# qinliuliuqin/Medical-Segmentation3d-Toolkit

Measured on AMD Instinct MI355X. Metric: patches/sec (96^3, 1-mod V-Net) train-step, higher is better.
Workload: dtype f32; 1 GPU; vnet(1,2) train step (fwd + Dice loss + bwd + fused Adam), 4 patches of 96^3 per GPU, fp32, random-init weights; global_batch=4, patch=96, parallelism=single GPU, wgrad_overlap=True, train_step_hipgraph=False, step_mode=auto, full=False

## Files before the change

### include/seg3d_hip.h

```cpp
#ifndef SEG3D_HIP_H
#define SEG3D_HIP_H

#ifdef __cplusplus
extern "C" {
#endif

#define SEG3D_ABI_VERSION 1

const char* seg3d_last_error(void);
int seg3d_abi_version(void);
const char* seg3d_target_arch(void);
int seg3d_device_count(void);

int seg3d_ncdhw_to_ndhwc(const float* in, float* out, int N, int C, long long S, void* stream);
int seg3d_ndhwc_to_ncdhw(const float* in, float* out, int N, int C, long long S, void* stream);
int seg3d_copy_channels(const float* src, float* dst, long long nvox, int C, int src_ld, int src_off, int dst_ld,
                        int dst_off, void* stream);

int seg3d_pack_weights_tapmajor(const float* w, float* wp, int A, int B, int BP, int T, long long sa, long long sb,
                                int flip, void* stream);
int seg3d_pack_weights_mfma(const float* w, float* wp, int A, int B, int T, long long sa, long long sb, int flip,
                            void* stream);
long long seg3d_packed_mfma_floats(int A, int B, int T);
typedef struct Seg3dPackJob {
// ... 152 lines not shown
                        int C, int relu, int ld_dout , void* stream);
int seg3d_gn_bwd_finalize(const float* part, const float* gamma, const float* mean_rstd, float* abx, float* s12,
                          float* dgamma, float* dbeta, float* dbias, int N, long long S, int C,
                          int acc_mask , void* stream);
int seg3d_gn_bwd_finalize_fused(const float* part, const float* gamma, const float* mean_rstd, float* abx, float* s12,
                                float* dgamma, float* dbeta, float* dbias, int* ticket, int N, long long S, int C,
                                int acc_mask, void* stream);
int seg3d_gn_bwd_apply(const float* dout, const float* out , const float* y, const float* mean_rstd,
                       const float* s12, const float* gamma, const float* beta, float* dy, float* dres, int N, long long S,
                       int C, int relu, int ld_dout , void* stream);

int seg3d_gn_mask_supported(int C);
int seg3d_gn_apply_mask(const float* y, const float* mean_rstd, const float* gamma, const float* beta, const float* res,
                        float* out, unsigned char* mask, int N, long long S, int C, int relu, int ld_out, void* stream);
int seg3d_gn_bwd_reduce_mask(const float* dout, const unsigned char* mask, const float* y, const float* mean_rstd,
                             float* part, int N, long long S, int C, int ld_dout, void* stream);
int seg3d_gn_bwd_apply_mask(const float* dout, const unsigned char* mask, const float* y, const float* mean_rstd,
                            const float* s12, const float* gamma, float* dy, float* dres ,
                            int N, long long S, int C, int ld_dout, void* stream);

int seg3d_gn_apply_mixed(const void* y, const float* mean_rstd, const float* gamma, const float* beta, const void* res,
                         void* out, int N, long long S, int C, int relu, int ld_out, int res_bf16, int out_bf16,
                         int y_bf16, void* stream);
int seg3d_gn_bwd_reduce_bf16(const void* dout_bf16, const void* out_bf16, const void* y, const float* mean_rstd,
                             const float* gamma, const float* beta, float* part, int N, long long S, int C, int relu,
                             int ld_dout, int y_bf16, void* stream);
int seg3d_gn_bwd_apply_bf16(const void* dout_bf16, const void* out_bf16, const void* y, const float* mean_rstd,
                            const float* s12, const float* gamma, const float* beta, void* dy, float* dres, int N,
                            long long S, int C, int relu, int ld_dout, int dy_bf16, int y_bf16, void* stream);

int seg3d_softmax_fwd(const float* in_ndhwc, float* probs_ncdhw, int N, int C, long long S, void* stream);
int seg3d_softmax_bwd(const float* probs_ncdhw, const float* dprobs_ncdhw, float* din_ndhwc, int N, int C, long long S,
                      void* stream);

long long seg3d_dice_blocks(long long S);
int seg3d_dice_fwd(const float* probs, const float* target, const float* weights, float* part, float* sums, float* loss,
                   int N, int C, long long S, void* stream);
int seg3d_dice_bwd(const float* probs, const float* target, const float* sums, const float* weights, const float* gout,
                   float* dprobs, int N, int C, long long S, void* stream);
int seg3d_binary_dice_fwd(const float* probs, const float* target, const float* one, float* part, float* sums, float* loss,
                          int N, long long S, void* stream);
int seg3d_binary_dice_bwd(const float* probs, const float* target, const float* sums, const float* gout, float* dprobs,
                          int N, long long S, void* stream);
long long seg3d_focal_blocks(long long total_vox);
int seg3d_focal_fwd(const float* probs, const float* target, const float* alpha, float* part, float* loss, int N, int C,
                    long long S, long long sn, long long sc, long long ss, float gamma, int size_average, void* stream);
int seg3d_focal_bwd(const float* probs, const float* target, const float* alpha, const float* gout, float* dprobs, int N,
                    int C, long long S, long long sn, long long sc, long long ss, float gamma, int size_average,
                    void* stream);
long long seg3d_compound_loss_part_floats(int N, int C, long long S);
int seg3d_compound_loss_fwd(const float* probs, const float* target, const float* wdice, const float* alpha, float* part,
                            float* coef, float* loss, int N, int C, long long S, float gamma, float dice_weight,
                            float ce_weight, int batch_dice, float ignore_label, void* stream);
int seg3d_compound_loss_bwd(const float* probs, const float* target, const float* coef, const float* alpha,
                            const float* gout, float* dprobs, int N, int C, long long S, float gamma, int batch_dice,
                            float ignore_label, void* stream);

int seg3d_sigmoid_fwd(const float* in_ndhwc, float* probs_ncdhw, int N, int C, long long S, void* stream);
int seg3d_sigmoid_bwd(const float* probs_ncdhw, const float* dprobs_ncdhw, float* din_ndhwc, int N, int C, long long S,
                      void* stream);

int seg3d_ds_head_supported(int Cin, int C);
int seg3d_ds_head_fwd(const float* x, int ldx, const float* w, const float* b, float* probs, int N, long long S, int Cin,
                      int C, void* stream);
long long seg3d_ds_head_bwd_workspace_floats(int N, long long S, int Cin, int C);
int seg3d_ds_head_bwd(const float* probs, const float* dprobs, const float* x, int ldx, const float* w, float* dx, int ld_dx,
// ... 130 lines not shown
```

### medical-segmentation3d-toolkit_amd/segmentation3d/_engine.py

```python
import ctypes
import os

import torch

_HERE = os.path.dirname(os.path.abspath(__file__))
_PKG_ROOT = os.path.dirname(_HERE)
LIB_PATH = os.environ.get('SEG3D_HIP_LIB', os.path.join(_PKG_ROOT, 'lib', 'libseg3d_hip.so'))

_c_int, _c_ll, _c_f, _c_p = ctypes.c_int, ctypes.c_longlong, ctypes.c_float, ctypes.c_void_p


class Normalizer(ctypes.Structure):
    _fields_ = [('type', _c_int), ('mean', _c_f), ('stddev', _c_f), ('clip', _c_int), ('clip_lo', _c_f), ('clip_hi', _c_f)]


class Normalizers(ctypes.Structure):
    _fields_ = [('n', Normalizer * 8)]



class Intensity(ctypes.Structure):
    _fields_ = [('brightness', _c_f), ('contrast', _c_f), ('gamma', _c_f), ('invert', _c_int), ('sigma', _c_f)]


# ... 110 lines not shown
    'seg3d_conv3d_k3_wino2d_wgrad_supported': (_c_int, [_c_int] * 6),
    'seg3d_conv3d_k3_wino2d_wgrad_preferred': (_c_int, [_c_int] * 6),
    'seg3d_conv3d_k3_wino2d_wgrad_workspace_floats': (_c_ll, [_c_int] * 6),
    'seg3d_conv3d_k3_wino2d_wgrad': (_c_int, [_c_p] * 4 + [_c_int] * 7 + [_c_p]),
    'seg3d_conv3d_k3_wino_wgrad_supported': (_c_int, [_c_int] * 6),
    'seg3d_conv3d_k3_wino_wgrad_workspace_floats': (_c_ll, [_c_int] * 6),
    'seg3d_conv3d_k3_wino_wgrad': (_c_int, [_c_p] * 4 + [_c_int] * 7 + [_c_p]),
    'seg3d_conv3d_k3_thin_out_f32mfma_supported': (_c_int, [_c_int] * 2),
    'seg3d_thin_out_f32mfma_packed_floats': (_c_ll, [_c_int] * 2),
    'seg3d_pack_weights_thin_out_f32mfma': (_c_int, [_c_p, _c_p, _c_int, _c_int, _c_ll, _c_ll, _c_int, _c_p]),
    'seg3d_conv3d_k3_thin_out_f32mfma_stats_count': (_c_ll, [_c_int] * 4),
    'seg3d_conv3d_k3_thin_out_f32mfma_fwd': (_c_int, [_c_p] * 5 + [_c_int] * 6 + [_c_p]),
    'seg3d_pack_weights_thin_out': (_c_int, [_c_p, _c_p, _c_int, _c_int, _c_int, _c_ll, _c_ll, _c_int, _c_p]),
    'seg3d_conv3d_k3_thin_out_stats_count': (_c_ll, [_c_int] * 3),
    'seg3d_conv3d_k3_thin_out_fwd': (_c_int, [_c_p] * 5 + [_c_int] * 7 + [_c_p]),
    'seg3d_k3_thin_wgrad_workspace_floats': (_c_ll, [_c_int] * 6),
    'seg3d_k3_thin_wgrad': (_c_int, [_c_p] * 4 + [_c_int] * 6 + [_c_ll, _c_ll, _c_int, _c_int, _c_p]),
    'seg3d_k3_thin_wgrad_fatbf16': (_c_int, [_c_p] * 4 + [_c_int] * 6 + [_c_ll, _c_ll, _c_int, _c_int, _c_p]),
    'seg3d_gn_stats_count': (_c_ll, [_c_ll]),
    'seg3d_gn_stats_partial': (_c_int, [_c_p, _c_p, _c_int, _c_ll, _c_p]),
    'seg3d_gn_stats_finalize': (_c_int, [_c_p, _c_p, _c_int, _c_int, _c_ll, _c_f, _c_p]),
    'seg3d_gn_apply': (_c_int, [_c_p] * 6 + [_c_int, _c_ll, _c_int, _c_int, _c_int, _c_p]),
    'seg3d_gn_bwd_blocks': (_c_ll, [_c_ll]),
    'seg3d_gn_bwd_reduce': (_c_int, [_c_p] * 7 + [_c_int, _c_ll, _c_int, _c_int, _c_int, _c_p]),
    'seg3d_gn_bwd_finalize': (_c_int, [_c_p] * 8 + [_c_int, _c_ll, _c_int, _c_int, _c_p]),
    'seg3d_gn_bwd_finalize_fused': (_c_int, [_c_p] * 9 + [_c_int, _c_ll, _c_int, _c_int, _c_p]),
    'seg3d_gn_bwd_apply': (_c_int, [_c_p] * 9 + [_c_int, _c_ll, _c_int, _c_int, _c_int, _c_p]),
    'seg3d_gn_mask_supported': (_c_int, [_c_int]),
    'seg3d_gn_apply_mask': (_c_int, [_c_p] * 7 + [_c_int, _c_ll, _c_int, _c_int, _c_int, _c_p]),
    'seg3d_gn_bwd_reduce_mask': (_c_int, [_c_p] * 5 + [_c_int, _c_ll, _c_int, _c_int, _c_p]),
    'seg3d_gn_bwd_apply_mask': (_c_int, [_c_p] * 8 + [_c_int, _c_ll, _c_int, _c_int, _c_p]),
    'seg3d_softmax_fwd': (_c_int, [_c_p, _c_p, _c_int, _c_int, _c_ll, _c_p]),
    'seg3d_softmax_bwd': (_c_int, [_c_p, _c_p, _c_p, _c_int, _c_int, _c_ll, _c_p]),
    'seg3d_dice_blocks': (_c_ll, [_c_ll]),
    'seg3d_dice_fwd': (_c_int, [_c_p] * 6 + [_c_int, _c_int, _c_ll, _c_p]),
    'seg3d_dice_bwd': (_c_int, [_c_p] * 6 + [_c_int, _c_int, _c_ll, _c_p]),
    'seg3d_binary_dice_fwd': (_c_int, [_c_p] * 6 + [_c_int, _c_ll, _c_p]),
    'seg3d_binary_dice_bwd': (_c_int, [_c_p] * 5 + [_c_int, _c_ll, _c_p]),
    'seg3d_focal_blocks': (_c_ll, [_c_ll]),
    'seg3d_focal_fwd': (_c_int, [_c_p] * 5 + [_c_int, _c_int, _c_ll, _c_ll, _c_ll, _c_ll, _c_f, _c_int, _c_p]),
    'seg3d_focal_bwd': (_c_int, [_c_p] * 5 + [_c_int, _c_int, _c_ll, _c_ll, _c_ll, _c_ll, _c_f, _c_int, _c_p]),
    'seg3d_compound_loss_part_floats': (_c_ll, [_c_int, _c_int, _c_ll]),
    'seg3d_compound_loss_fwd': (_c_int, [_c_p] * 7 + [_c_int, _c_int, _c_ll, _c_f, _c_f, _c_f, _c_int, _c_f, _c_p]),
    'seg3d_compound_loss_bwd': (_c_int, [_c_p] * 6 + [_c_int, _c_int, _c_ll, _c_f, _c_int, _c_f, _c_p]),
    'seg3d_sigmoid_fwd': (_c_int, [_c_p, _c_p, _c_int, _c_int, _c_ll, _c_p]),
    'seg3d_sigmoid_bwd': (_c_int, [_c_p, _c_p, _c_p, _c_int, _c_int, _c_ll, _c_p]),
    'seg3d_ds_head_supported': (_c_int, [_c_int] * 2),
    'seg3d_ds_head_fwd': (_c_int, [_c_p, _c_int, _c_p, _c_p, _c_p, _c_int, _c_ll, _c_int, _c_int, _c_p]),
    'seg3d_ds_head_bwd_workspace_floats': (_c_ll, [_c_int, _c_ll, _c_int, _c_int]),
    'seg3d_ds_head_bwd': (_c_int, [_c_p] * 3 + [_c_int, _c_p, _c_p, _c_int, _c_p, _c_int, _c_ll, _c_int, _c_int, _c_p]),
    'seg3d_ds_head_bwd_finalize': (_c_int, [_c_p] * 3 + [_c_int, _c_ll, _c_int, _c_int, _c_int, _c_p]),
    'seg3d_label_pyramid': (_c_int, [_c_p] * 4 + [_c_int] * 5 + [_c_p]),
    'seg3d_adam_step': (_c_int, [_c_p] * 4 + [_c_ll, _c_int] + [_c_f] * 6 + [_c_p]),
    'seg3d_adam_step_devstep': (_c_int, [_c_p] * 4 + [_c_ll, _c_p, _c_p] + [_c_f] * 6 + [_c_p]),
    'seg3d_grad_sumsq_part_count': (_c_ll, [_c_ll]),
    'seg3d_grad_sumsq_partial': (_c_int, [_c_p, _c_ll, _c_p, _c_p]),
    'seg3d_optim_prepare': (_c_int, [_c_p, _c_p, _c_p, _c_int, _c_f, _c_f, _c_int, _c_f, _c_int, _c_int, _c_f, _c_f, _c_f,
                                     _c_p]),
    'seg3d_sgd_step_ctl': (_c_int, [_c_p, _c_p, _c_p, _c_ll, _c_p, _c_f, _c_f, _c_int, _c_p]),
    'seg3d_adam_step_ctl': (_c_int, [_c_p] * 4 + [_c_ll, _c_p] + [_c_f] * 4 + [_c_p]),
    'seg3d_patch_stats_blocks': (_c_ll, [_c_int] * 3),
    'seg3d_patch_gather_normalize': (_c_int, [_c_p] * 5 + [_c_int] * 8 + [_c_f, _c_f, _c_int, _c_f, _c_p]),
    'seg3d_patch_stats_mc_doubles': (_c_ll, [_c_int] * 5),
    'seg3d_patch_gather_normalize_mc': (_c_int, [_c_p] * 5 + [_c_int] * 8 + [Normalizers, _c_p]),
    'seg3d_patch_scatter_accumulate': (_c_int, [_c_p] * 5 + [_c_int] * 7 + [_c_ll, _c_p]),
    'seg3d_finalize_argmax': (_c_int, [_c_p, _c_p, _c_p, _c_int, _c_ll, _c_ll, _c_p]),
# ... 102 lines not shown
```

### medical-segmentation3d-toolkit_amd/segmentation3d/_ops.py

```python
import contextlib
import ctypes

import torch

from . import _engine as E
from . import _grad_sink as G

GN_EPS = 1e-5

_KINDS = {'k3': (3, 1, 27, False), 'k2s2': (2, 2, 8, False), 'k1': (1, 1, 1, False), 'convT': (2, 2, 8, True)}

FORCE_DIRECT = False
WINOGRAD = True
WINOGRAD2D = True
STREAM_K = True
_TWO_FORWARDS = 0
RELU_MASK = True


@contextlib.contextmanager
def two_forwards():
    global _TWO_FORWARDS
    _TWO_FORWARDS += 1
    try:
# ... 623 lines not shown
               E.ptr(mask), N, D * H * W_, C, int(relu), ld, E.stream_ptr())
        return out
    if _is_bf16(out) or _is_bf16(resn) or _is_bf16(yn):
        E.call('seg3d_gn_apply_mixed', E.ptr(yn), E.ptr(mean_rstd), E.ptr(gamma), E.ptr(beta), E.ptr(resn), E.ptr(out), N,
               D * H * W_, C, int(relu), ld, int(_is_bf16(resn)), int(_is_bf16(out)), int(_is_bf16(yn)), E.stream_ptr())
        return out
    E.call('seg3d_gn_apply', E.ptr(yn), E.ptr(mean_rstd), E.ptr(gamma), E.ptr(beta), E.ptr(resn), E.ptr(out), N,
           D * H * W_, C, int(relu), ld, E.stream_ptr())
    return out


def _row_stride(t, C):
    if t.is_contiguous():
        return 0
    N, D, H, W_, _ = t.shape
    ld = t.stride(3)
    if t.stride(4) != 1 or ld < C or ld % 4 or t.stride(2) != W_ * ld or t.stride(1) != H * t.stride(2) or \
            t.stride(0) != D * t.stride(1) or (t.storage_offset() % 4):
        raise ValueError('expected a contiguous NDHWC tensor or a channel slice of one')
    return ld


GN_FUSED_FINALIZE = False
_GN_TICKETS = {}


def _gn_ticket(device):
    t = _GN_TICKETS.get(device)
    if t is None:
        t = _GN_TICKETS[device] = torch.zeros(1, dtype=torch.int32, device=device)
    return t


def gn_backward(doutn, outn, yn, mean_rstd, gamma, beta, relu, want_dres, want_dbias=True, sinks=(None, None, None),
                dy_bf16=False, mask=None):
    N, D, H, W_, C = yn.shape
    S = D * H * W_
    nblk = E.query('seg3d_gn_bwd_blocks', S)
    part = _empty((N, nblk, C, 3), yn)
    mask_src = outn if relu else None
    ldd = _row_stride(doutn, C)
    act_bf16 = _is_bf16(doutn)
    if act_bf16 != (_is_bf16(mask_src) if mask_src is not None else act_bf16):
        raise TypeError('GroupNorm backward: gradient and saved output differ in dtype')
    if dy_bf16 and not act_bf16:
        raise TypeError('GroupNorm backward: a bf16 conv gradient needs a bf16 unit output')
    if _is_bf16(yn) and not act_bf16:
        yn = _to_f32(yn)
    y16 = int(_is_bf16(yn))
    if mask is not None:
        if not relu or outn is not None or act_bf16 or y16 or mask.dtype != torch.uint8 or not mask.is_contiguous() or \
                mask.numel() * 4 != yn.numel():
            raise ValueError('GroupNorm backward: the ReLU mask belongs to a fp32 ReLU unit and stands in for its output')
        E.call('seg3d_gn_bwd_reduce_mask', E.ptr(doutn), E.ptr(mask), E.ptr(yn), E.ptr(mean_rstd), E.ptr(part), N, S, C, ldd,
               E.stream_ptr())
    elif act_bf16:
        E.call('seg3d_gn_bwd_reduce_bf16', E.ptr(doutn), E.ptr(mask_src), E.ptr(yn), E.ptr(mean_rstd), E.ptr(gamma),
               E.ptr(beta), E.ptr(part), N, S, C, int(relu), ldd, y16, E.stream_ptr())
    else:
        E.call('seg3d_gn_bwd_reduce', E.ptr(doutn), E.ptr(mask_src), E.ptr(yn), E.ptr(mean_rstd), E.ptr(gamma),
               E.ptr(beta), E.ptr(part), N, S, C, int(relu), ldd, E.stream_ptr())
    abx = _empty((N, C, 3), yn)
    s12 = _empty((N, 2), yn)
    sg, sb_, sc = sinks
    for t in sinks:
        if t is not None and (t.numel() != C or not t.is_contiguous()):
            raise ValueError('GroupNorm gradient destination must be a contiguous [C] tensor')
    dgamma = _empty((C,), yn) if sg is None else sg
    dbeta = _empty((C,), yn) if sb_ is None else sb_
    dbias = (_empty((C,), yn) if sc is None else sc) if want_dbias else None
    acc_mask = (1 if sg is not None else 0) | (2 if sb_ is not None else 0) | (4 if (want_dbias and sc is not None) else 0)
    if GN_FUSED_FINALIZE:
        E.call('seg3d_gn_bwd_finalize_fused', E.ptr(part), E.ptr(gamma), E.ptr(mean_rstd), E.ptr(abx), E.ptr(s12),
               E.ptr(dgamma), E.ptr(dbeta), E.ptr(dbias), E.ptr(_gn_ticket(yn.device)), N, S, C, acc_mask, E.stream_ptr())
    else:
        E.call('seg3d_gn_bwd_finalize', E.ptr(part), E.ptr(gamma), E.ptr(mean_rstd), E.ptr(abx), E.ptr(s12), E.ptr(dgamma),
               E.ptr(dbeta), E.ptr(dbias), N, S, C, acc_mask, E.stream_ptr())
    dy = torch.empty(yn.shape, dtype=torch.bfloat16 if dy_bf16 else torch.float32, device=yn.device)
    dres = torch.empty(yn.shape, dtype=torch.float32, device=yn.device) if want_dres else None
    if mask is not None:
        E.call('seg3d_gn_bwd_apply_mask', E.ptr(doutn), E.ptr(mask), E.ptr(yn), E.ptr(mean_rstd), E.ptr(s12), E.ptr(gamma),
               E.ptr(dy), E.ptr(dres), N, S, C, ldd, E.stream_ptr())
    elif act_bf16:
        E.call('seg3d_gn_bwd_apply_bf16', E.ptr(doutn), E.ptr(mask_src), E.ptr(yn), E.ptr(mean_rstd), E.ptr(s12),
               E.ptr(gamma), E.ptr(beta), E.ptr(dy), E.ptr(dres), N, S, C, int(relu), ldd, int(dy_bf16), y16,
               E.stream_ptr())
    else:
        E.call('seg3d_gn_bwd_apply', E.ptr(doutn), E.ptr(mask_src), E.ptr(yn), E.ptr(mean_rstd), E.ptr(s12), E.ptr(gamma),
               E.ptr(beta), E.ptr(dy), E.ptr(dres), N, S, C, int(relu), ldd, E.stream_ptr())
    return (dy, dres, dgamma if sg is None else None, dbeta if sb_ is None else None,
            dbias if (want_dbias and sc is None) else None)


WGRAD_SIDE_STREAM = True
_SIDE_STREAMS = {}
_SIDE_STREAMS_UNPROBED = {}
SIDE_KEEPALIVE = True
_SIDE_KEEP = {}
_JOIN_QUEUED_FOR = [-1]


def _runs_beside(busy, other, spin_cycles=1500000):
    probe = torch.zeros(1024, device=busy.device)
    votes = 0
    for _ in range(3):
        torch.cuda.synchronize()
        s0, e_busy, e_other = (torch.cuda.Event(enable_timing=True) for _ in range(3))
        s0.record(busy)
        other.wait_event(s0)
        with torch.cuda.stream(busy):
            torch.cuda._sleep(spin_cycles)
        e_busy.record(busy)
        with torch.cuda.stream(other):
            probe.add_(1.0)
        e_other.record(other)
        torch.cuda.synchronize()
        votes += int(s0.elapsed_time(e_other) < 0.5 * s0.elapsed_time(e_busy))
    return votes >= 2


def _side_stream(device):
    st = _SIDE_STREAMS.get(device.index)
    if st is None:
        with torch.cuda.device(device):
# ... 331 lines not shown
        return da, db


def cat_channels(a, b):
    return CatChannelsFunction.apply(a, b)


class SoftmaxFunction(torch.autograd.Function):

    @staticmethod
    def forward(ctx, x):
        E.require_device(x)
        xn = to_ndhwc(x)
        N, D, H, W_, C = xn.shape
        probs = _empty((N, C, D, H, W_), xn)
        E.call('seg3d_softmax_fwd', E.ptr(xn), E.ptr(probs), N, C, D * H * W_, E.stream_ptr())
        ctx.save_for_backward(probs)
        return probs

    @staticmethod
    def backward(ctx, dprobs):
        (probs,) = ctx.saved_tensors
        N, C, D, H, W_ = probs.shape
        dp = dprobs.contiguous()
        din = _empty((N, D, H, W_, C), probs)
        E.call('seg3d_softmax_bwd', E.ptr(probs), E.ptr(dp), E.ptr(din), N, C, D * H * W_, E.stream_ptr())
        return from_ndhwc(din)


def softmax_channels(x):
    return SoftmaxFunction.apply(x)


class SigmoidFunction(torch.autograd.Function):

    @staticmethod
    def forward(ctx, x):
        E.require_device(x)
        if x.dtype != torch.float32:
            raise ValueError('the sigmoid head takes float32 logits, got {} (bf16 activation mode supports up to 15 '
                             'regions)'.format(x.dtype))
        xn = to_ndhwc(x)
        N, D, H, W_, C = xn.shape
        probs = _empty((N, C, D, H, W_), xn)
        E.call('seg3d_sigmoid_fwd', E.ptr(xn), E.ptr(probs), N, C, D * H * W_, E.stream_ptr())
        ctx.save_for_backward(probs)
        return probs

    @staticmethod
    def backward(ctx, dprobs):
        (probs,) = ctx.saved_tensors
        N, C, D, H, W_ = probs.shape
        dp = dprobs.contiguous()
        din = _empty((N, D, H, W_, C), probs)
        E.call('seg3d_sigmoid_bwd', E.ptr(probs), E.ptr(dp), E.ptr(din), N, C, D * H * W_, E.stream_ptr())
        return from_ndhwc(din)


def sigmoid_channels(x):
    return SigmoidFunction.apply(x)


class DiceLossFunction(torch.autograd.Function):

    @staticmethod
    def forward(ctx, probs, target, weights):
# ... 229 lines not shown
```

### medical-segmentation3d-toolkit_amd/segmentation3d/network/module/vnet_outblock.py

```python
import torch.nn as nn

from segmentation3d.network.module.layers import Sigmoid, Softmax, attach_unit, run_unit

_FIRST, _SECOND = ('conv1', 'gn1', 'act1'), ('conv2', 'gn2', None)
ACTIVATIONS = ('softmax', 'sigmoid')


def check_activation(activation):
    if activation not in ACTIVATIONS:
        raise ValueError("unknown output activation {!r}: 'softmax' or 'sigmoid'".format(activation))
    return activation


class OutputBlock(nn.Module):

    def __init__(self, in_channels, out_channels, activation='softmax'):
        super(OutputBlock, self).__init__()
        self.activation = check_activation(activation)
        attach_unit(self, _FIRST, 'k3', in_channels, out_channels)
        attach_unit(self, _SECOND, 'k1', out_channels, out_channels, act=False)
        if self.activation == 'sigmoid':
            self.sigmoid = Sigmoid()
        else:
            self.softmax = Softmax(dim=1)

    def forward(self, input):
        hidden = run_unit(self, _FIRST, input, relu=True)
        logits = run_unit(self, _SECOND, hidden, relu=False)
        return self.sigmoid(logits) if self.activation == 'sigmoid' else self.softmax(logits)
```

Measured before the change: 286.4 patches/s.

## Fuse V-Net output block GN/ReLU/1x1 conv/GN/softmax into custom head-tail kernels

Adds HIP kernels that fuse the output block's tail (GN1 apply + ReLU, 1x1 conv, GN2 stats/apply, softmax) and its backward into a few streaming passes. Intermediate activations are recomputed from y1 rather than stored. The aim is to cut memory traffic and kernel launches at full resolution. The cost is extra recompute in each backward pass and extra code paths, limited to at most 8 classes in fp32.

```diff
diff --git a/include/seg3d_hip.h b/include/seg3d_hip.h
--- a/include/seg3d_hip.h
+++ b/include/seg3d_hip.h
@@ -208,6 +208,24 @@
 int seg3d_softmax_fwd(const float* in_ndhwc, float* probs_ncdhw, int N, int C, long long S, void* stream);
 int seg3d_softmax_bwd(const float* probs_ncdhw, const float* dprobs_ncdhw, float* din_ndhwc, int N, int C, long long S,
                       void* stream);
+
+long long seg3d_head_tail_blocks(long long S);
+int seg3d_head_tail_stats(const float* y1, const float* mean_rstd1, const float* gamma1, const float* beta1, const float* w2,
+                          const float* b2, float* stats_partial, int N, long long S, int C, void* stream);
+int seg3d_head_tail_fwd(const float* y1, const float* mean_rstd1, const float* gamma1, const float* beta1, const float* w2,
+                        const float* b2, const float* mean_rstd2, const float* gamma2, const float* beta2, float* probs, int N,
+                        long long S, int C, void* stream);
+int seg3d_head_tail_bwd_stats2(const float* probs, const float* dprobs, const float* y1, const float* mean_rstd1,
+                               const float* gamma1, const float* beta1, const float* w2, const float* b2,
+                               const float* mean_rstd2, float* part2, int N, long long S, int C, void* stream);
+int seg3d_head_tail_bwd_stats1(const float* probs, const float* dprobs, const float* y1, const float* mean_rstd1,
+                               const float* gamma1, const float* beta1, const float* w2, const float* b2,
+                               const float* mean_rstd2, const float* gamma2, const float* s12_2, float* part1, float* wpart,
+                               float* dw2, int N, long long S, int C, int accumulate, void* stream);
+int seg3d_head_tail_bwd_apply(const float* probs, const float* dprobs, const float* y1, const float* mean_rstd1,
+                              const float* gamma1, const float* beta1, const float* w2, const float* b2,
+                              const float* mean_rstd2, const float* gamma2, const float* s12_2, const float* s12_1, float* dy1,
+                              int N, long long S, int C, void* stream);
 
 long long seg3d_dice_blocks(long long S);
 int seg3d_dice_fwd(const float* probs, const float* target, const float* weights, float* part, float* sums, float* loss,
diff --git a/medical-segmentation3d-toolkit_amd/csrc/head_tail.hip b/medical-segmentation3d-toolkit_amd/csrc/head_tail.hip
--- /dev/null
+++ b/medical-segmentation3d-toolkit_amd/csrc/head_tail.hip
@@ -0,0 +1,517 @@
+#include "seg3d_common.h"
+#include "seg3d_hip.h"
+
+#define HT_MAXC 8
+
+template <int C>
+struct HtUnit {
+  float mean1, rstd1, g1[C], b1[C];
+  float w2[C][C], bias2[C];
+  float mean2, rstd2, g2[C], b2[C];
+  __device__ __forceinline__ void load1(const float* __restrict__ mr1, const float* __restrict__ gamma1,
+                                        const float* __restrict__ beta1, const float* __restrict__ w,
+                                        const float* __restrict__ bias, int n) {
+    mean1 = mr1[2 * n], rstd1 = mr1[2 * n + 1];
+#pragma unroll
+    for (int k = 0; k < C; ++k) {
+      g1[k] = gamma1[k], b1[k] = beta1[k];
+      bias2[k] = bias ? bias[k] : 0.f;
+#pragma unroll
+      for (int j = 0; j < C; ++j) w2[k][j] = w[k * C + j];
+    }
+  }
+  __device__ __forceinline__ void load2(const float* __restrict__ mr2, const float* __restrict__ gamma2,
+                                        const float* __restrict__ beta2, int n) {
+    mean2 = mr2[2 * n], rstd2 = mr2[2 * n + 1];
+#pragma unroll
+    for (int c = 0; c < C; ++c) g2[c] = gamma2 ? gamma2[c] : 1.f, b2[c] = beta2 ? beta2[c] : 0.f;
+  }
+};
+
+template <int C>
+__device__ __forceinline__ void ht_a1(const HtUnit<C>& u, const float (&y)[C], float (&a1)[C]) {
+#pragma unroll
+  for (int k = 0; k < C; ++k) a1[k] = fmaxf((y[k] - u.mean1) * u.rstd1 * u.g1[k] + u.b1[k], 0.f);
+}
+template <int C>
+__device__ __forceinline__ void ht_z(const HtUnit<C>& u, const float (&a1)[C], float (&z)[C]) {
+#pragma unroll
+  for (int c = 0; c < C; ++c) z[c] = u.bias2[c];
+#pragma unroll
+  for (int k = 0; k < C; ++k)
+#pragma unroll
+    for (int c = 0; c < C; ++c) z[c] = fmaf(a1[k], u.w2[c][k], z[c]);
+}
+template <int C>
+__device__ __forceinline__ void ht_probs(const HtUnit<C>& u, const float (&z)[C], float (&p)[C]) {
+  float mx = -INFINITY;
+#pragma unroll
+  for (int c = 0; c < C; ++c) {
+    p[c] = (z[c] - u.mean2) * u.rstd2 * u.g2[c] + u.b2[c];
+    mx = fmaxf(mx, p[c]);
+  }
+  float sum = 0.f;
+#pragma unroll
+  for (int c = 0; c < C; ++c) {
+    p[c] = expf(p[c] - mx);
+    sum += p[c];
+  }
+#pragma unroll
+  for (int c = 0; c < C; ++c) p[c] = p[c] / sum;
+}
+template <int C>
+__device__ __forceinline__ void ht_dzn(const float (&p)[C], const float (&dp)[C], float (&dzn)[C]) {
+  float dot = 0.f;
+#pragma unroll
+  for (int c = 0; c < C; ++c) dot += p[c] * dp[c];
+#pragma unroll
+  for (int c = 0; c < C; ++c) dzn[c] = p[c] * (dp[c] - dot);
+}
+template <int C>
+__device__ __forceinline__ void ht_dz(const HtUnit<C>& u, const float (&z)[C], const float (&dzn)[C], float s1, float s2,
+                                      float (&dz)[C]) {
+#pragma unroll
+  for (int c = 0; c < C; ++c) dz[c] = u.rstd2 * (u.g2[c] * dzn[c] - s1 - (z[c] - u.mean2) * u.rstd2 * s2);
+}
+template <int C>
+__device__ __forceinline__ void ht_g1(const HtUnit<C>& u, const float (&a1)[C], const float (&dz)[C], float (&g1)[C]) {
+#pragma unroll
+  for (int k = 0; k < C; ++k) g1[k] = 0.f;
+#pragma unroll
+  for (int c = 0; c < C; ++c)
+#pragma unroll
+    for (int k = 0; k < C; ++k) g1[k] = fmaf(dz[c], u.w2[c][k], g1[k]);
+#pragma unroll
+  for (int k = 0; k < C; ++k) g1[k] = a1[k] > 0.f ? g1[k] : 0.f;
+}
+
+template <int C, bool VEC>
+__device__ __forceinline__ void ht_load_rows(const float* __restrict__ p, int nv, float (&v)[4][C]) {
+  if (VEC) {
+#pragma unroll
+    for (int i = 0; i < C; ++i) {
+      const seg3d_f32x4 t = __builtin_nontemporal_load(reinterpret_cast<const seg3d_f32x4*>(p) + i);
+#pragma unroll
+      for (int j = 0; j < 4; ++j) v[(4 * i + j) / C][(4 * i + j) % C] = t[j];
+    }
+  } else {
+#pragma unroll
+    for (int j = 0; j < 4; ++j)
+#pragma unroll
+      for (int c = 0; c < C; ++c) v[j][c] = j < nv ? p[j * C + c] : 0.f;
+  }
+}
+template <int C, bool VEC>
+__device__ __forceinline__ void ht_store_rows(float* __restrict__ p, int nv, const float (&v)[4][C]) {
+  if (VEC) {
+#pragma unroll
+    for (int i = 0; i < C; ++i) {
+      seg3d_f32x4 t;
+#pragma unroll
+      for (int j = 0; j < 4; ++j) t[j] = v[(4 * i + j) / C][(4 * i + j) % C];
+      __builtin_nontemporal_store(t, reinterpret_cast<seg3d_f32x4*>(p) + i);
+    }
+  } else {
+#pragma unroll
+    for (int j = 0; j < 4; ++j)
+#pragma unroll
+      for (int c = 0; c < C; ++c)
+        if (j < nv) p[j * C + c] = v[j][c];
+  }
+}
+template <int C, bool VEC>
+__device__ __forceinline__ void ht_load_planes(const float* __restrict__ p, i64 S, int nv, float (&v)[4][C]) {
+#pragma unroll
+  for (int c = 0; c < C; ++c) {
+    if (VEC) {
+      const seg3d_f32x4 t = __builtin_nontemporal_load(reinterpret_cast<const seg3d_f32x4*>(p + c * S));
+#pragma unroll
+      for (int j = 0; j < 4; ++j) v[j][c] = t[j];
+    } else {
+#pragma unroll
+      for (int j = 0; j < 4; ++j) v[j][c] = j < nv ? p[c * S + j] : 0.f;
+    }
+  }
+}
+template <int C, bool VEC>
+__device__ __forceinline__ void ht_store_planes(float* __restrict__ p, i64 S, int nv, const float (&v)[4][C]) {
+#pragma unroll
+  for (int c = 0; c < C; ++c) {
+    if (VEC) {
+      const seg3d_f32x4 t = {v[0][c], v[1][c], v[2][c], v[3][c]};
+      __builtin_nontemporal_store(t, reinterpret_cast<seg3d_f32x4*>(p + c * S));
+    } else {
+#pragma unroll
+      for (int j = 0; j < 4; ++j)
+        if (j < nv) p[c * S + j] = v[j][c];
+    }
+  }
+}
+
+struct HtRange {
+  i64 q0, q1;
+  __device__ __forceinline__ HtRange(i64 S, int qpb) {
+    const i64 Q = (S + 3) >> 2;
+    q0 = (i64)blockIdx.x * qpb;
+    q1 = q0 + qpb < Q ? q0 + qpb : Q;
+  }
+};
+template <bool VEC>
+__device__ __forceinline__ int ht_nvalid(i64 S, i64 s) {
+  return VEC ? 4 : (S - s < 4 ? (int)(S - s) : 4);
+}
+
+template <int NV>
+__device__ __forceinline__ void ht_block_sum(float (&v)[NV], double* red) {
+  const int lane = threadIdx.x & 63, wave = threadIdx.x >> 6;
+#pragma unroll
+  for (int k = 0; k < NV; ++k) {
+    const double w = wave_sum_d((double)v[k]);
+    if (lane == 0) red[wave * NV + k] = w;
+  }
+  __syncthreads();
+  if (threadIdx.x == 0) {
+#pragma unroll
+    for (int k = 0; k < NV; ++k) v[k] = (float)((red[k] + red[NV + k]) + (red[2 * NV + k] + red[3 * NV + k]));
+  }
+}
+
+template <int C, bool VEC>
+__global__ __launch_bounds__(256) void head_tail_stats_kernel(const float* __restrict__ y1, const float* __restrict__ mr1,
+                                                                const float* __restrict__ gamma1,
+                                                                const float* __restrict__ beta1, const float* __restrict__ w2,
+                                                                const float* __restrict__ bias2, float* __restrict__ part,
+                                                                i64 S, int qpb) {
+  __shared__ double red[4 * 2];
+  const int n = blockIdx.y;
+  HtUnit<C> u;
+  u.load1(mr1, gamma1, beta1, w2, bias2, n);
+  const HtRange r(S, qpb);
+  float acc[2] = {0.f, 0.f};
+  for (i64 q = r.q0 + threadIdx.x; q < r.q1; q += 256) {
+    const i64 s = 4 * q;
+    const int nv = ht_nvalid<VEC>(S, s);
+    float y[4][C];
+    ht_load_rows<C, VEC>(y1 + ((i64)n * S + s) * C, nv, y);
+#pragma unroll
+    for (int j = 0; j < 4; ++j) {
+      float a1[C], z[C];
+      ht_a1<C>(u, y[j], a1);
+      ht_z<C>(u, a1, z);
+      if (j < nv) {
+#pragma unroll
+        for (int c = 0; c < C; ++c) {
+          acc[0] += z[c];
+          acc[1] += z[c] * z[c];
+        }
+      }
+    }
+  }
+  ht_block_sum<2>(acc, red);
+  if (threadIdx.x == 0) {
+    float* dst = part + ((i64)n * gridDim.x + blockIdx.x) * 2;
+    dst[0] = acc[0];
+    dst[1] = acc[1];
+  }
+}
+
+template <int C, bool VEC>
+__global__ __launch_bounds__(256) void head_tail_fwd_kernel(const float* __restrict__ y1, const float* __restrict__ mr1,
+                                                              const float* __restrict__ gamma1, const float* __restrict__ beta1,
+                                                              const float* __restrict__ w2, const float* __restrict__ bias2,
+                                                              const float* __restrict__ mr2, const float* __restrict__ gamma2,
+                                                              const float* __restrict__ beta2, float* __restrict__ probs, i64 S,
+                                                              int qpb) {
+  const int n = blockIdx.y;
+  HtUnit<C> u;
+  u.load1(mr1, gamma1, beta1, w2, bias2, n);
+  u.load2(mr2, gamma2, beta2, n);
+  const HtRange r(S, qpb);
+  for (i64 q = r.q0 + threadIdx.x; q < r.q1; q += 256) {
+    const i64 s = 4 * q;
+    const int nv = ht_nvalid<VEC>(S, s);
+    float y[4][C], p[4][C];
+    ht_load_rows<C, VEC>(y1 + ((i64)n * S + s) * C, nv, y);
+#pragma unroll
+    for (int j = 0; j < 4; ++j) {
+      float a1[C], z[C];
+      ht_a1<C>(u, y[j], a1);
+      ht_z<C>(u, a1, z);
+      ht_probs<C>(u, z, p[j]);
+    }
+    ht_store_planes<C, VEC>(probs + (i64)n * C * S + s, S, nv, p);
+  }
+}
+
+template <int C, bool VEC>
+__global__ __launch_bounds__(256) void head_tail_bwd_stats2_kernel(const float* __restrict__ probs,
+                                                                     const float* __restrict__ dprobs,
+                                                                     const float* __restrict__ y1, const float* __restrict__ mr1,
+                                                                     const float* __restrict__ gamma1,
+                                                                     const float* __restrict__ beta1, const float* __restrict__ w2,
+                                                                     const float* __restrict__ bias2, const float* __restrict__ mr2,
+                                                                     float* __restrict__ part2, i64 S, int qpb) {
+  __shared__ double red[4 * 3 * C];
+  const int n = blockIdx.y;
+  HtUnit<C> u;
+  u.load1(mr1, gamma1, beta1, w2, bias2, n);
+  u.load2(mr2, nullptr, nullptr, n);
+  const HtRange r(S, qpb);
+  float acc[3 * C];
+#pragma unroll
+  for (int k = 0; k < 3 * C; ++k) acc[k] = 0.f;
+  for (i64 q = r.q0 + threadIdx.x; q < r.q1; q += 256) {
+    const i64 s = 4 * q;
+    const int nv = ht_nvalid<VEC>(S, s);
+    float y[4][C], p[4][C], dp[4][C];
+    ht_load_rows<C, VEC>(y1 + ((i64)n * S + s) * C, nv, y);
+    ht_load_planes<C, VEC>(probs + (i64)n * C * S + s, S, nv, p);
+    ht_load_planes<C, VEC>(dprobs + (i64)n * C * S + s, S, nv, dp);
+#pragma unroll
+    for (int j = 0; j < 4; ++j) {
+      float a1[C], z[C], dzn[C];
+      ht_a1<C>(u, y[j], a1);
+      ht_z<C>(u, a1, z);
+      ht_dzn<C>(p[j], dp[j], dzn);
+      if (j < nv) {
+#pragma unroll
+        for (int c = 0; c < C; ++c) {
+          const float zh = (z[c] - u.mean2) * u.rstd2;
+          acc[3 * c + 0] += dzn[c];
+          acc[3 * c + 1] += dzn[c] * zh;
+          acc[3 * c + 2] += zh;
+        }
+      }
+    }
+  }
+  ht_block_sum<3 * C>(acc, red);
+  if (threadIdx.x == 0) {
+    float* dst = part2 + ((i64)n * gridDim.x + blockIdx.x) * C * 3;
+#pragma unroll
+    for (int k = 0; k < 3 * C; ++k) dst[k] = acc[k];
+  }
+}
+
+template <int C, bool VEC>
+__global__ __launch_bounds__(256) void head_tail_bwd_stats1_kernel(const float* __restrict__ probs,
+                                                                     const float* __restrict__ dprobs,
+                                                                     const float* __restrict__ y1, const float* __restrict__ mr1,
+                                                                     const float* __restrict__ gamma1,
+                                                                     const float* __restrict__ beta1, const float* __restrict__ w2,
+                                                                     const float* __restrict__ bias2, const float* __restrict__ mr2,
+                                                                     const float* __restrict__ gamma2,
+                                                                     const float* __restrict__ s12_2, float* __restrict__ part1,
+                                                                     float* __restrict__ wpart, i64 S, int qpb) {
+  constexpr int NV = 3 * C + C * C;
+  __shared__ double red[4 * NV];
+  const int n = blockIdx.y;
+  HtUnit<C> u;
+  u.load1(mr1, gamma1, beta1, w2, bias2, n);
+  u.load2(mr2, gamma2, nullptr, n);
+  const float s1 = s12_2[2 * n], s2 = s12_2[2 * n + 1];
+  const HtRange r(S, qpb);
+  float acc[NV];
+#pragma unroll
+  for (int k = 0; k < NV; ++k) acc[k] = 0.f;
+  for (i64 q = r.q0 + threadIdx.x; q < r.q1; q += 256) {
+    const i64 s = 4 * q;
+    const int nv = ht_nvalid<VEC>(S, s);
+    float y[4][C], p[4][C], dp[4][C];
+    ht_load_rows<C, VEC>(y1 + ((i64)n * S + s) * C, nv, y);
+    ht_load_planes<C, VEC>(probs + (i64)n * C * S + s, S, nv, p);
+    ht_load_planes<C, VEC>(dprobs + (i64)n * C * S + s, S, nv, dp);
+#pragma unroll
+    for (int j = 0; j < 4; ++j) {
+      float a1[C], z[C], dzn[C], dz[C], g1[C];
+      ht_a1<C>(u, y[j], a1);
+      ht_z<C>(u, a1, z);
+      ht_dzn<C>(p[j], dp[j], dzn);
+      ht_dz<C>(u, z, dzn, s1, s2, dz);
+      ht_g1<C>(u, a1, dz, g1);
+      if (j < nv) {
+#pragma unroll
+        for (int k = 0; k < C; ++k) {
+          const float xh = (y[j][k] - u.mean1) * u.rstd1;
+          acc[3 * k + 0] += g1[k];
+          acc[3 * k + 1] += g1[k] * xh;
+          acc[3 * k + 2] += xh;
+        }
+#pragma unroll
+        for (int c = 0; c < C; ++c)
+#pragma unroll
+          for (int k = 0; k < C; ++k) acc[3 * C + c * C + k] += dz[c] * a1[k];
+      }
+    }
+  }
+  ht_block_sum<NV>(acc, red);
+  if (threadIdx.x == 0) {
+    const i64 slot = (i64)n * gridDim.x + blockIdx.x;
+    float* d1 = part1 + slot * C * 3;
+#pragma unroll
+    for (int k = 0; k < 3 * C; ++k) d1[k] = acc[k];
+    float* dw = wpart + slot * (C * C);
+#pragma unroll
+    for (int k = 0; k < C * C; ++k) dw[k] = acc[3 * C + k];
+  }
+}
+
+__global__ __launch_bounds__(256) void head_tail_wreduce_kernel(const float* __restrict__ wpart, float* __restrict__ dw2,
+                                                                  int slots, int NV, int accumulate) {
+  __shared__ double red[256];
+  const int o = blockIdx.x;
+  double s = 0.0;
+  for (int k = threadIdx.x; k < slots; k += 256) s += (double)wpart[(i64)k * NV + o];
+  red[threadIdx.x] = s;
+  __syncthreads();
+#pragma unroll
+  for (int w = 128; w >= 1; w >>= 1) {
+    if ((int)threadIdx.x < w) red[threadIdx.x] += red[threadIdx.x + w];
+    __syncthreads();
+  }
+  if (threadIdx.x == 0) {
+    const float v = (float)red[0];
+    dw2[o] = accumulate ? dw2[o] + v : v;
+  }
+}
+
+template <int C, bool VEC>
+__global__ __launch_bounds__(256) void head_tail_bwd_apply_kernel(const float* __restrict__ probs,
+                                                                    const float* __restrict__ dprobs,
+                                                                    const float* __restrict__ y1, const float* __restrict__ mr1,
+                                                                    const float* __restrict__ gamma1,
+                                                                    const float* __restrict__ beta1, const float* __restrict__ w2,
+                                                                    const float* __restrict__ bias2, const float* __restrict__ mr2,
+                                                                    const float* __restrict__ gamma2,
+                                                                    const float* __restrict__ s12_2,
+                                                                    const float* __restrict__ s12_1, float* __restrict__ dy1,
+                                                                    i64 S, int qpb) {
+  const int n = blockIdx.y;
+  HtUnit<C> u;
+  u.load1(mr1, gamma1, beta1, w2, bias2, n);
+  u.load2(mr2, gamma2, nullptr, n);
+  const float s1 = s12_2[2 * n], s2 = s12_2[2 * n + 1];
+  const float t1 = s12_1[2 * n], t2 = s12_1[2 * n + 1];
+  const HtRange r(S, qpb);
+  for (i64 q = r.q0 + threadIdx.x; q < r.q1; q += 256) {
+    const i64 s = 4 * q;
+    const int nv = ht_nvalid<VEC>(S, s);
+    float y[4][C], p[4][C], dp[4][C], dy[4][C];
+    ht_load_rows<C, VEC>(y1 + ((i64)n * S + s) * C, nv, y);
+    ht_load_planes<C, VEC>(probs + (i64)n * C * S + s, S, nv, p);
+    ht_load_planes<C, VEC>(dprobs + (i64)n * C * S + s, S, nv, dp);
+#pragma unroll
+    for (int j = 0; j < 4; ++j) {
+      float a1[C], z[C], dzn[C], dz[C], g1[C];
+      ht_a1<C>(u, y[j], a1);
+      ht_z<C>(u, a1, z);
+      ht_dzn<C>(p[j], dp[j], dzn);
+      ht_dz<C>(u, z, dzn, s1, s2, dz);
+      ht_g1<C>(u, a1, dz, g1);
+#pragma unroll
+      for (int k = 0; k < C; ++k) dy[j][k] = u.rstd1 * (u.g1[k] * g1[k] - t1 - (y[j][k] - u.mean1) * u.rstd1 * t2);
+    }
+    ht_store_rows<C, VEC>(dy1 + ((i64)n * S + s) * C, nv, dy);
+  }
+}
+
+extern "C" long long seg3d_head_tail_blocks(long long S) { return seg3d_gn_bwd_blocks(S); }
+
+static inline int ht_qpb(i64 S, int nblk) { return (int)((((S + 3) >> 2) + nblk - 1) / nblk); }
+static inline bool ht_aligned(const void* p) { return (reinterpret_cast<unsigned long long>(p) & 15) == 0; }
+
+#define HT_CASE(KERNEL, CC, ...)                                                                             \
+  case CC:                                                                                                   \
+    if (vec) hipLaunchKernelGGL((KERNEL<CC, true>), grid, dim3(256), 0, s, __VA_ARGS__);                     \
+    else hipLaunchKernelGGL((KERNEL<CC, false>), grid, dim3(256), 0, s, __VA_ARGS__);                        \
+    break;
+#define HT_LAUNCH(KERNEL, ...)                                                                               \
+  switch (C) {                                                                                               \
+    HT_CASE(KERNEL, 1, __VA_ARGS__) HT_CASE(KERNEL, 2, __VA_ARGS__) HT_CASE(KERNEL, 3, __VA_ARGS__)          \
+    HT_CASE(KERNEL, 4, __VA_ARGS__) HT_CASE(KERNEL, 5, __VA_ARGS__) HT_CASE(KERNEL, 6, __VA_ARGS__)          \
+    HT_CASE(KERNEL, 7, __VA_ARGS__) HT_CASE(KERNEL, 8, __VA_ARGS__)                                          \
+  }
+#define HT_REQUIRE_SHAPE(name)                                                                               \
+  SEG3D_REQUIRE(N > 0 && N <= 65535 && S > 0, name ": bad arguments");                                       \
+  SEG3D_REQUIRE(C >= 1 && C <= HT_MAXC, name ": classes %d not in [1, %d]", C, HT_MAXC)
+
+extern "C" int seg3d_head_tail_stats(const float* y1, const float* mean_rstd1, const float* gamma1, const float* beta1,
+                                     const float* w2, const float* b2, float* stats_partial, int N, long long S, int C,
+                                     void* stream) {
+  SEG3D_REQUIRE(y1 && mean_rstd1 && gamma1 && beta1 && w2 && stats_partial, "seg3d_head_tail_stats: bad arguments");
+  HT_REQUIRE_SHAPE("seg3d_head_tail_stats");
+  const int nblk = (int)seg3d_head_tail_blocks(S), qpb = ht_qpb(S, nblk);
+  const bool vec = (S & 3) == 0 && ht_aligned(y1);
+  const dim3 grid(nblk, N);
+  hipStream_t s = (hipStream_t)stream;
+  HT_LAUNCH(head_tail_stats_kernel, y1, mean_rstd1, gamma1, beta1, w2, b2, stats_partial, (i64)S, qpb)
+  SEG3D_LAUNCH_CHECK("seg3d_head_tail_stats");
+  return SEG3D_OK;
+}
+
+extern "C" int seg3d_head_tail_fwd(const float* y1, const float* mean_rstd1, const float* gamma1, const float* beta1,
+                                   const float* w2, const float* b2, const float* mean_rstd2, const float* gamma2,
+                                   const float* beta2, float* probs, int N, long long S, int C, void* stream) {
+  SEG3D_REQUIRE(y1 && mean_rstd1 && gamma1 && beta1 && w2 && mean_rstd2 && gamma2 && beta2 && probs,
+                "seg3d_head_tail_fwd: bad arguments");
+  HT_REQUIRE_SHAPE("seg3d_head_tail_fwd");
+  const int nblk = (int)seg3d_head_tail_blocks(S), qpb = ht_qpb(S, nblk);
+  const bool vec = (S & 3) == 0 && ht_aligned(y1) && ht_aligned(probs);
+  const dim3 grid(nblk, N);
+  hipStream_t s = (hipStream_t)stream;
+  HT_LAUNCH(head_tail_fwd_kernel, y1, mean_rstd1, gamma1, beta1, w2, b2, mean_rstd2, gamma2, beta2, probs, (i64)S, qpb)
+  SEG3D_LAUNCH_CHECK("seg3d_head_tail_fwd");
+  return SEG3D_OK;
+}
+
+extern "C" int seg3d_head_tail_bwd_stats2(const float* probs, const float* dprobs, const float* y1, const float* mean_rstd1,
+                                          const float* gamma1, const float* beta1, const float* w2, const float* b2,
+                                          const float* mean_rstd2, float* part2, int N, long long S, int C, void* stream) {
+  SEG3D_REQUIRE(probs && dprobs && y1 && mean_rstd1 && gamma1 && beta1 && w2 && mean_rstd2 && part2,
+                "seg3d_head_tail_bwd_stats2: bad arguments");
+  HT_REQUIRE_SHAPE("seg3d_head_tail_bwd_stats2");
+  const int nblk = (int)seg3d_head_tail_blocks(S), qpb = ht_qpb(S, nblk);
+  const bool vec = (S & 3) == 0 && ht_aligned(y1) && ht_aligned(probs) && ht_aligned(dprobs);
+  const dim3 grid(nblk, N);
+  hipStream_t s = (hipStream_t)stream;
+  HT_LAUNCH(head_tail_bwd_stats2_kernel, probs, dprobs, y1, mean_rstd1, gamma1, beta1, w2, b2, mean_rstd2, part2, (i64)S, qpb)
+  SEG3D_LAUNCH_CHECK("seg3d_head_tail_bwd_stats2");
+  return SEG3D_OK;
+}
+
+extern "C" int seg3d_head_tail_bwd_stats1(const float* probs, const float* dprobs, const float* y1, const float* mean_rstd1,
+                                          const float* gamma1, const float* beta1, const float* w2, const float* b2,
+                                          const float* mean_rstd2, const float* gamma2, const float* s12_2, float* part1,
+                                          float* wpart, float* dw2, int N, long long S, int C, int accumulate,
+                                          void* stream) {
+  SEG3D_REQUIRE(probs && dprobs && y1 && mean_rstd1 && gamma1 && beta1 && w2 && mean_rstd2 && gamma2 && s12_2 && part1 &&
+                    wpart && dw2,
+                "seg3d_head_tail_bwd_stats1: bad arguments");
+  HT_REQUIRE_SHAPE("seg3d_head_tail_bwd_stats1");
+  const int nblk = (int)seg3d_head_tail_blocks(S), qpb = ht_qpb(S, nblk);
+  const bool vec = (S & 3) == 0 && ht_aligned(y1) && ht_aligned(probs) && ht_aligned(dprobs);
+  const dim3 grid(nblk, N);
+  hipStream_t s = (hipStream_t)stream;
+  HT_LAUNCH(head_tail_bwd_stats1_kernel, probs, dprobs, y1, mean_rstd1, gamma1, beta1, w2, b2, mean_rstd2, gamma2, s12_2, part1,
+            wpart, (i64)S, qpb)
+  SEG3D_LAUNCH_CHECK("seg3d_head_tail_bwd_stats1");
+  hipLaunchKernelGGL(head_tail_wreduce_kernel, dim3(C * C), dim3(256), 0, s, wpart, dw2, N * nblk, C * C, accumulate);
+  SEG3D_LAUNCH_CHECK("seg3d_head_tail_bwd_stats1(reduce)");
+  return SEG3D_OK;
+}
+
+extern "C" int seg3d_head_tail_bwd_apply(const float* probs, const float* dprobs, const float* y1, const float* mean_rstd1,
+                                         const float* gamma1, const float* beta1, const float* w2, const float* b2,
+                                         const float* mean_rstd2, const float* gamma2, const float* s12_2, const float* s12_1,
+                                         float* dy1, int N, long long S, int C, void* stream) {
+  SEG3D_REQUIRE(probs && dprobs && y1 && mean_rstd1 && gamma1 && beta1 && w2 && mean_rstd2 && gamma2 && s12_2 && s12_1 && dy1,
+                "seg3d_head_tail_bwd_apply: bad arguments");
+  HT_REQUIRE_SHAPE("seg3d_head_tail_bwd_apply");
+  const int nblk = (int)seg3d_head_tail_blocks(S), qpb = ht_qpb(S, nblk);
+  const bool vec = (S & 3) == 0 && ht_aligned(y1) && ht_aligned(probs) && ht_aligned(dprobs) && ht_aligned(dy1);
+  const dim3 grid(nblk, N);
+  hipStream_t s = (hipStream_t)stream;
+  HT_LAUNCH(head_tail_bwd_apply_kernel, probs, dprobs, y1, mean_rstd1, gamma1, beta1, w2, b2, mean_rstd2, gamma2, s12_2, s12_1,
+            dy1, (i64)S, qpb)
+  SEG3D_LAUNCH_CHECK("seg3d_head_tail_bwd_apply");
+  return SEG3D_OK;
+}
diff --git a/medical-segmentation3d-toolkit_amd/segmentation3d/_engine.py b/medical-segmentation3d-toolkit_amd/segmentation3d/_engine.py
--- a/medical-segmentation3d-toolkit_amd/segmentation3d/_engine.py
+++ b/medical-segmentation3d-toolkit_amd/segmentation3d/_engine.py
@@ -166,6 +166,12 @@
     'seg3d_gn_bwd_apply_mask': (_c_int, [_c_p] * 8 + [_c_int, _c_ll, _c_int, _c_int, _c_p]),
     'seg3d_softmax_fwd': (_c_int, [_c_p, _c_p, _c_int, _c_int, _c_ll, _c_p]),
     'seg3d_softmax_bwd': (_c_int, [_c_p, _c_p, _c_p, _c_int, _c_int, _c_ll, _c_p]),
+    'seg3d_head_tail_blocks': (_c_ll, [_c_ll]),
+    'seg3d_head_tail_stats': (_c_int, [_c_p] * 7 + [_c_int, _c_ll, _c_int, _c_p]),
+    'seg3d_head_tail_fwd': (_c_int, [_c_p] * 10 + [_c_int, _c_ll, _c_int, _c_p]),
+    'seg3d_head_tail_bwd_stats2': (_c_int, [_c_p] * 10 + [_c_int, _c_ll, _c_int, _c_p]),
+    'seg3d_head_tail_bwd_stats1': (_c_int, [_c_p] * 14 + [_c_int, _c_ll, _c_int, _c_int, _c_p]),
+    'seg3d_head_tail_bwd_apply': (_c_int, [_c_p] * 13 + [_c_int, _c_ll, _c_int, _c_p]),
     'seg3d_dice_blocks': (_c_ll, [_c_ll]),
     'seg3d_dice_fwd': (_c_int, [_c_p] * 6 + [_c_int, _c_int, _c_ll, _c_p]),
     'seg3d_dice_bwd': (_c_int, [_c_p] * 6 + [_c_int, _c_int, _c_ll, _c_p]),
diff --git a/medical-segmentation3d-toolkit_amd/segmentation3d/_ops.py b/medical-segmentation3d-toolkit_amd/segmentation3d/_ops.py
--- a/medical-segmentation3d-toolkit_amd/segmentation3d/_ops.py
+++ b/medical-segmentation3d-toolkit_amd/segmentation3d/_ops.py
@@ -679,6 +679,27 @@
     return t
 
 
+def _gn_bwd_finalize(part, gamma, mean_rstd, N, S, C, want_dbias, sinks):
+    abx = _empty((N, C, 3), part)
+    s12 = _empty((N, 2), part)
+    sg, sb_, sc = sinks
+    for t in sinks:
+        if t is not None and (t.numel() != C or not t.is_contiguous()):
+            raise ValueError('GroupNorm gradient destination must be a contiguous [C] tensor')
+    dgamma = _empty((C,), part) if sg is None else sg
+    dbeta = _empty((C,), part) if sb_ is None else sb_
+    dbias = (_empty((C,), part) if sc is None else sc) if want_dbias else None
+    acc_mask = (1 if sg is not None else 0) | (2 if sb_ is not None else 0) | (4 if (want_dbias and sc is not None) else 0)
+    if GN_FUSED_FINALIZE:
+        E.call('seg3d_gn_bwd_finalize_fused', E.ptr(part), E.ptr(gamma), E.ptr(mean_rstd), E.ptr(abx), E.ptr(s12),
+               E.ptr(dgamma), E.ptr(dbeta), E.ptr(dbias), E.ptr(_gn_ticket(part.device)), N, S, C, acc_mask, E.stream_ptr())
+    else:
+        E.call('seg3d_gn_bwd_finalize', E.ptr(part), E.ptr(gamma), E.ptr(mean_rstd), E.ptr(abx), E.ptr(s12), E.ptr(dgamma),
+               E.ptr(dbeta), E.ptr(dbias), N, S, C, acc_mask, E.stream_ptr())
+    return (s12, dgamma if sg is None else None, dbeta if sb_ is None else None,
+            dbias if (want_dbias and sc is None) else None)
+
+
 def gn_backward(doutn, outn, yn, mean_rstd, gamma, beta, relu, want_dres, want_dbias=True, sinks=(None, None, None),
                 dy_bf16=False, mask=None):
     N, D, H, W_, C = yn.shape
@@ -707,22 +728,7 @@
     else:
         E.call('seg3d_gn_bwd_reduce', E.ptr(doutn), E.ptr(mask_src), E.ptr(yn), E.ptr(mean_rstd), E.ptr(gamma),
                E.ptr(beta), E.ptr(part), N, S, C, int(relu), ldd, E.stream_ptr())
-    abx = _empty((N, C, 3), yn)
-    s12 = _empty((N, 2), yn)
-    sg, sb_, sc = sinks
-    for t in sinks:
-        if t is not None and (t.numel() != C or not t.is_contiguous()):
-            raise ValueError('GroupNorm gradient destination must be a contiguous [C] tensor')
-    dgamma = _empty((C,), yn) if sg is None else sg
-    dbeta = _empty((C,), yn) if sb_ is None else sb_
-    dbias = (_empty((C,), yn) if sc is None else sc) if want_dbias else None
-    acc_mask = (1 if sg is not None else 0) | (2 if sb_ is not None else 0) | (4 if (want_dbias and sc is not None) else 0)
-    if GN_FUSED_FINALIZE:
-        E.call('seg3d_gn_bwd_finalize_fused', E.ptr(part), E.ptr(gamma), E.ptr(mean_rstd), E.ptr(abx), E.ptr(s12),
-               E.ptr(dgamma), E.ptr(dbeta), E.ptr(dbias), E.ptr(_gn_ticket(yn.device)), N, S, C, acc_mask, E.stream_ptr())
-    else:
-        E.call('seg3d_gn_bwd_finalize', E.ptr(part), E.ptr(gamma), E.ptr(mean_rstd), E.ptr(abx), E.ptr(s12), E.ptr(dgamma),
-               E.ptr(dbeta), E.ptr(dbias), N, S, C, acc_mask, E.stream_ptr())
+    s12, dgamma, dbeta, dbias = _gn_bwd_finalize(part, gamma, mean_rstd, N, S, C, want_dbias, sinks)
     dy = torch.empty(yn.shape, dtype=torch.bfloat16 if dy_bf16 else torch.float32, device=yn.device)
     dres = torch.empty(yn.shape, dtype=torch.float32, device=yn.device) if want_dres else None
     if mask is not None:
@@ -735,8 +741,7 @@
     else:
         E.call('seg3d_gn_bwd_apply', E.ptr(doutn), E.ptr(mask_src), E.ptr(yn), E.ptr(mean_rstd), E.ptr(s12), E.ptr(gamma),
                E.ptr(beta), E.ptr(dy), E.ptr(dres), N, S, C, int(relu), ldd, E.stream_ptr())
-    return (dy, dres, dgamma if sg is None else None, dbeta if sb_ is None else None,
-            dbias if (want_dbias and sc is None) else None)
+    return dy, dres, dgamma, dbeta, dbias
 
 
 WGRAD_SIDE_STREAM = True
@@ -1134,6 +1139,101 @@
     return SoftmaxFunction.apply(x)
 
 
+HEAD_TAIL_FUSED = True
+HEAD_TAIL_MAX_CLASSES = 8
+
+
+def head_tail_usable(x, classes):
+    return HEAD_TAIL_FUSED and not FORCE_DIRECT and not _ACT_BF16[0] and x.is_cuda and x.dtype == torch.float32 and \
+        1 <= classes <= HEAD_TAIL_MAX_CLASSES
+
+
+class ConvStatsFunction(torch.autograd.Function):
+
+    @staticmethod
+    def forward(ctx, x, weight, bias, kind, eps):
+        E.require_device(x, weight, bias)
+        xn = to_ndhwc(x)
+        w = weight.detach()
+        yn, partial = conv_forward(xn, w, None if bias is None else bias.detach(), kind, want_stats=True)
+        mean_rstd = gn_stats(yn, partial, eps)
+        ctx.kind, ctx.w_shape, ctx.sink = kind, tuple(weight.shape), G.lookup(weight)
+        ctx.save_for_backward(xn, w)
+        ctx.mark_non_differentiable(mean_rstd)
+        return from_ndhwc(yn), mean_rstd
+
+    @staticmethod
+    def backward(ctx, dy, _dstats):
+        xn, w = ctx.saved_tensors
+        dyn = to_ndhwc(dy)
+        dx = from_ndhwc(conv_dgrad(dyn, w, ctx.kind, want_bf16=_is_bf16(xn))) if ctx.needs_input_grad[0] else None
+        dw = None
+        if ctx.needs_input_grad[1]:
+            if ctx.sink is not None:
+                _wgrad_to_sink(xn, dyn, ctx.w_shape, ctx.kind, ctx.sink.view)
+            else:
+                dw = conv_wgrad(xn, dyn, ctx.w_shape, ctx.kind)
+        return dx, dw, None, None, None
+
+
+def conv_stats(x, weight, bias, kind='k3', eps=GN_EPS):
+    return ConvStatsFunction.apply(x, weight, bias, kind, eps)
+
+
+def _head_tail_blocks(S):
+    return E.query('seg3d_head_tail_blocks', S)
+
+
+class HeadTailFunction(torch.autograd.Function):
+
+    @staticmethod
+    def forward(ctx, y1, mean_rstd1, bias1, gamma1, beta1, weight2, bias2, gamma2, beta2, eps):
+        E.require_device(y1, mean_rstd1, bias1, gamma1, beta1, weight2, bias2, gamma2, beta2)
+        yn = to_ndhwc(y1)
+        N, D, H, W_, C = yn.shape
+        S = D * H * W_
+        _check_w(weight2, (C, C, 1, 1, 1), 'k1')
+        g1, b1, w2, g2, b2 = (t.detach() for t in (gamma1, beta1, weight2, gamma2, beta2))
+        c2 = None if bias2 is None else bias2.detach()
+        part = _empty((N, _head_tail_blocks(S), 2), yn)
+        E.call('seg3d_head_tail_stats', E.ptr(yn), E.ptr(mean_rstd1), E.ptr(g1), E.ptr(b1), E.ptr(w2), E.ptr(c2), E.ptr(part), N,
+               S, C, E.stream_ptr())
+        mean_rstd2 = gn_stats(yn, part, eps)
+        probs = _empty((N, C, D, H, W_), yn)
+        E.call('seg3d_head_tail_fwd', E.ptr(yn), E.ptr(mean_rstd1), E.ptr(g1), E.ptr(b1), E.ptr(w2), E.ptr(c2),
+               E.ptr(mean_rstd2), E.ptr(g2), E.ptr(b2), E.ptr(probs), N, S, C, E.stream_ptr())
+        ctx.has_bias1, ctx.has_bias2 = bias1 is not None, bias2 is not None
+        ctx.sinks = tuple(G.lookup(t) for t in (bias1, gamma1, beta1, weight2, bias2, gamma2, beta2))
+        ctx.save_for_backward(yn, mean_rstd1, mean_rstd2, probs, g1, b1, w2, c2, g2)
+        return probs
+
+    @staticmethod
+    def backward(ctx, dprobs):
+        yn, mr1, mr2, probs, g1, b1, w2, c2, g2 = ctx.saved_tensors
+        N, D, H, W_, C = yn.shape
+        S = D * H * W_
+        nblk = _head_tail_blocks(S)
+        s_c1, s_g1, s_b1, s_w2, s_c2, s_g2, s_b2 = _views(*ctx.sinks)
+        dp = dprobs.contiguous()
+        head = (E.ptr(probs), E.ptr(dp), E.ptr(yn), E.ptr(mr1), E.ptr(g1), E.ptr(b1), E.ptr(w2), E.ptr(c2), E.ptr(mr2))
+        part2 = _empty((N, nblk, C, 3), yn)
+        E.call('seg3d_head_tail_bwd_stats2', *head, E.ptr(part2), N, S, C, E.stream_ptr())
+        s12_2, dgamma2, dbeta2, db2 = _gn_bwd_finalize(part2, g2, mr2, N, S, C, ctx.has_bias2, (s_g2, s_b2, s_c2))
+        part1 = _empty((N, nblk, C, 3), yn)
+        wpart = _empty((N, nblk, C * C), yn)
+        dw2 = _empty((C, C, 1, 1, 1), yn) if s_w2 is None else s_w2
+        E.call('seg3d_head_tail_bwd_stats1', *head, E.ptr(g2), E.ptr(s12_2), E.ptr(part1), E.ptr(wpart), E.ptr(dw2), N, S, C,
+               int(s_w2 is not None), E.stream_ptr())
+        s12_1, dgamma1, dbeta1, dbias1 = _gn_bwd_finalize(part1, g1, mr1, N, S, C, ctx.has_bias1, (s_g1, s_b1, s_c1))
+        dy1 = _empty(yn.shape, yn)
+        E.call('seg3d_head_tail_bwd_apply', *head, E.ptr(g2), E.ptr(s12_2), E.ptr(s12_1), E.ptr(dy1), N, S, C, E.stream_ptr())
+        return (from_ndhwc(dy1), None, dbias1, dgamma1, dbeta1, dw2 if s_w2 is None else None, db2, dgamma2, dbeta2, None)
+
+
+def head_tail(y1, mean_rstd1, bias1, gamma1, beta1, weight2, bias2, gamma2, beta2, eps=GN_EPS):
+    return HeadTailFunction.apply(y1, mean_rstd1, bias1, gamma1, beta1, weight2, bias2, gamma2, beta2, eps)
+
+
 class SigmoidFunction(torch.autograd.Function):
 
     @staticmethod
diff --git a/medical-segmentation3d-toolkit_amd/segmentation3d/network/module/vnet_outblock.py b/medical-segmentation3d-toolkit_amd/segmentation3d/network/module/vnet_outblock.py
--- a/medical-segmentation3d-toolkit_amd/segmentation3d/network/module/vnet_outblock.py
+++ b/medical-segmentation3d-toolkit_amd/segmentation3d/network/module/vnet_outblock.py
@@ -1,5 +1,6 @@
 import torch.nn as nn
 
+from segmentation3d import _ops
 from segmentation3d.network.module.layers import Sigmoid, Softmax, attach_unit, run_unit
 
 _FIRST, _SECOND = ('conv1', 'gn1', 'act1'), ('conv2', 'gn2', None)
@@ -25,6 +26,10 @@
             self.softmax = Softmax(dim=1)
 
     def forward(self, input):
+        if self.activation == 'softmax' and _ops.head_tail_usable(input, self.conv2.out_channels):
+            y1, mean_rstd1 = _ops.conv_stats(input, self.conv1.weight, self.conv1.bias, kind=self.conv1.kind, eps=self.gn1.eps)
+            return _ops.head_tail(y1, mean_rstd1, self.conv1.bias, self.gn1.weight, self.gn1.bias, self.conv2.weight,
+                                  self.conv2.bias, self.gn2.weight, self.gn2.bias, eps=self.gn2.eps)
         hidden = run_unit(self, _FIRST, input, relu=True)
         logits = run_unit(self, _SECOND, hidden, relu=False)
         return self.sigmoid(logits) if self.activation == 'sigmoid' else self.softmax(logits)
```

Result: no change. 288.4 patches/s, median of 6 (+0.7%).
